# GAVLab/feature_extraction

Measured on AMD Instinct MI355X. Metric: VLP-16 scans/sec (16x1800 pts), detector+descriptor, higher is better.
Workload: dtype f32; 1 GPU; batch of 1024 synthetic VLP-16 scans (16x1800 pts, 64 uniform poles) per GPU, device-resident, preset 'launch', roll/pitch 0.02/-0.015; scans_per_gpu=1024, preset=launch, parallelism=frame-sharded x1, batches_in_flight=4

## Files before the change

feature_extraction_amd/csrc/fx_kernels.hip:

```cpp
#include <hip/hip_runtime.h>
#include <float.h>
#include <math.h>
#include <assert.h>
#include <type_traits>
#include <algorithm>

#include "fx_device.h"
#include "fx_sort_replay.h"
#include "fx_launch.h"
#include "../../include/fx.h"

#pragma clang fp contract(off)

#define FX_WG 256
#define FX_NWAVE (FX_WG / 64)

namespace {

typedef float fx_f2 __attribute__((ext_vector_type(2)));

__device__ __forceinline__ uint32_t lanes_below(unsigned long long m) {
  return __builtin_amdgcn_mbcnt_hi((uint32_t)(m >> 32), __builtin_amdgcn_mbcnt_lo((uint32_t)m, 0u));
}

// ... 3841 lines not shown
  for (uint32_t k = tid; k < K; k += NT) {
    const float4 kp = B.keypoints[(size_t)G.scan * G.P.max_keypoints + G.kb + k];
    s.kp[k] = kp;
    s.kcnt[k] = 0;
    s.kpos[k] = 0;
    s.knbr[k] = 0;
    if (G.slice == 0 && MODE != 1) B.row_kp[G.row0 + k] = kp;
    atomicMin(&s.w[GW_BOX + 0], f2ord(kp.x)), atomicMax(&s.w[GW_BOX + 1], f2ord(kp.x));
    atomicMin(&s.w[GW_BOX + 2], f2ord(kp.y)), atomicMax(&s.w[GW_BOX + 3], f2ord(kp.y));
    atomicMin(&s.w[GW_BOX + 4], f2ord(kp.z)), atomicMax(&s.w[GW_BOX + 5], f2ord(kp.z));
  }
  __syncthreads();
  GatherGrid g;
  const float kx0 = ord2f(s.w[GW_BOX + 0]), kx1 = ord2f(s.w[GW_BOX + 1]), ky0 = ord2f(s.w[GW_BOX + 2]), ky1 = ord2f(s.w[GW_BOX + 3]);
  g.bx0 = kx0 - box_margin, g.bx1 = kx1 + box_margin;
  g.by0 = ky0 - box_margin, g.by1 = ky1 + box_margin;
  g.bz0 = ord2f(s.w[GW_BOX + 4]) - box_margin, g.bz1 = ord2f(s.w[GW_BOX + 5]) + box_margin;
  const float wx = fmaxf(box_margin, (g.bx1 - g.bx0) / (float)(FX_GATHER_G - 1) * 1.0001f + 1e-6f);
  const float wy = fmaxf(box_margin, (g.by1 - g.by0) / (float)(FX_GATHER_G - 1) * 1.0001f + 1e-6f);
  g.inv_wx = 1.0f / wx, g.inv_wy = 1.0f / wy;
  g.ncx = min((int)((g.bx1 - g.bx0) * g.inv_wx) + 1, FX_GATHER_G), g.ncy = min((int)((g.by1 - g.by0) * g.inv_wy) + 1, FX_GATHER_G);
  const int ncx = g.ncx, ncy = g.ncy;
  for (uint32_t k = tid; k < K; k += NT) {
    const int cx = g.cell_x(s.kp[k].x), cy = g.cell_y(s.kp[k].y);
    for (int dy = -1; dy <= 1; ++dy)
      for (int dx = -1; dx <= 1; ++dx)
        if (cx + dx >= 0 && cx + dx < ncx && cy + dy >= 0 && cy + dy < ncy) atomicAdd(&s.cell[(cy + dy) * ncx + cx + dx], 1u);
  }
  __syncthreads();
  if (tid < 64) {
    const uint32_t n_cells = (uint32_t)(ncx * ncy), per = (n_cells + 63) / 64;
    uint32_t sum = 0;
    for (uint32_t u = 0; u < per; ++u) {
      const uint32_t ci = tid * per + u;
      sum += ci < n_cells ? s.cell[ci] : 0u;
    }
    uint32_t incl = sum;
    incl = wave_incl_scan(incl);
    uint32_t run = incl - sum;
    for (uint32_t u = 0; u < per; ++u) {
      const uint32_t ci = tid * per + u;
      if (ci < n_cells) {
        const uint32_t c = s.cell[ci];
        s.cell[ci] = run | (c << 20);
        s.cur[ci] = run;
        run += c;
      }
    }
  }
  __syncthreads();
  for (uint32_t k = tid; k < K; k += NT) {
    const int cx = g.cell_x(s.kp[k].x), cy = g.cell_y(s.kp[k].y);
    for (int dy = -1; dy <= 1; ++dy)
      for (int dx = -1; dx <= 1; ++dx)
        if (cx + dx >= 0 && cx + dx < ncx && cy + dy >= 0 && cy + dy < ncy)
          s.flat[atomicAdd(&s.cur[(cy + dy) * ncx + cx + dx], 1u)] = (uint16_t)k;
  }
  __syncthreads();
  return g;
}
template <int NT>
__device__ __forceinline__ void gather_slice_positions(const GatherWg &G) {
  const uint32_t S = gridDim.x;
  const uint32_t *cnt = G.B.gather_cnt + (size_t)G.scan * S * G.P.max_keypoints;
  uint32_t ovf_before = 0, ovf_all = 0;
  for (uint32_t k = G.tid; k < G.K; k += NT) {
    uint32_t run = 0, mine = 0;
    for (uint32_t sl = 0; sl < S; ++sl) {
      const uint32_t c = cnt[(size_t)sl * G.P.max_keypoints + k];
      const uint32_t o = run + c > G.P.list_cap ? run + c - max(run, G.P.list_cap) : 0u;
      if (sl == G.slice) mine = run;
      if (sl < G.slice) ovf_before += o;
      ovf_all += o;
      run += c;
    }
    G.s.kpos[k] = mine;
    if (G.slice == 0) G.B.s_cnt[G.row0 + k] = run;
  }
  if (ovf_before) atomicAdd(&G.s.w[GW_OVF], ovf_before);
  if (G.slice == 0 && ovf_all) atomicAdd(&G.B.ovf_cnt[G.scan], ovf_all);
  __syncthreads();
}
template <int NT, int MODE>
struct GatherStream {
  static constexpr uint32_t kTile = NT * 4;
  uint32_t lo, hi, tstep, nb_first;
  const uint32_t *near_bits;
  uint2 nb_words;
  __device__ __forceinline__ GatherStream(const GatherWg &G) {
    const uint32_t n = G.M.n;
    uint32_t chunk = (n + gridDim.x - 1) / gridDim.x;
    chunk = (chunk + kTile - 1) / kTile * kTile;
    tstep = MODE != 0 ? gridDim.x * kTile : kTile;
    lo = MODE != 0 ? G.slice * kTile : G.slice * chunk;
    hi = MODE != 0 ? n : (lo + chunk < n ? lo + chunk : n);
    near_bits = G.B.near_bits + (size_t)G.scan * G.P.near_words;
    nb_fill(G, lo);
  }
  __device__ __forceinline__ void nb_fill(const GatherWg &G, uint32_t i_first) {
    nb_first = i_first;
    const uint32_t i = i_first + G.lane * tstep;
    nb_words = make_uint2(0u, 0u);
    if (i < hi) {
      const uint32_t w = (i + G.wave * 256u) / 128u;
      nb_words = *reinterpret_cast<const uint2 *>(near_bits + w);
    }
  }
  __device__ __forceinline__ unsigned long long near_sectors(const GatherWg &G, uint32_t i0) {
    if (i0 >= hi) return 0ull;
    uint32_t t = (i0 - nb_first) / tstep;
    if (t >= 64u) nb_fill(G, i0), t = 0u;
    const uint32_t ts = (uint32_t)__builtin_amdgcn_readfirstlane((int)t);
    return (unsigned long long)(uint32_t)__builtin_amdgcn_readlane((int)nb_words.x, (int)ts) |
           ((unsigned long long)(uint32_t)__builtin_amdgcn_readlane((int)nb_words.y, (int)ts) << 32);
  }
  __device__ __forceinline__ void load_tile(const GatherWg &G, uint32_t i0, unsigned long long sect, float4 (&v)[4]) const {
#pragma unroll
    for (int u = 0; u < 4; ++u) {
      const uint32_t i = i0 + G.wave * 256 + u * 64 + G.lane;
      v[u] = make_float4(NAN, NAN, NAN, 0);
      if (((sect >> (16 * u + (G.lane >> 2))) & 1ull) && i < hi) v[u] = *reinterpret_cast<const float4 *>(G.M.pts + (size_t)i * G.M.stride_f);
    }
  }
};
__device__ __forceinline__ void hit_count(const GatherWg &G, uint32_t k) { atomicAdd(&G.s.kpos[k], 1u); }
__device__ __forceinline__ void hit_direct(const GatherWg &G, uint32_t k, const float4 &pq) {
  const uint32_t pos = G.own ? atomicAdd(&G.s.kpos[k], 1u) : atomicAdd(&G.B.s_cnt[G.row0 + k], 1u);
  if (pos < G.P.list_cap) {
    G.B.s_pts[(size_t)(G.row0 + k) * G.P.list_cap + pos] = pq;
  } else {
    const uint32_t os = G.own ? atomicAdd(&G.s.w[GW_OVF], 1u) : atomicAdd(&G.B.ovf_cnt[G.scan], 1u);
    if (os < G.P.ovf_cap) {
      G.ovf_pts[os] = pq;
      G.ovf_kp[os] = k;
    }
  }
}
__device__ __forceinline__ bool hit_staged(const GatherWg &G, uint32_t k, const float4 &pq) {
  const uint32_t slot = atomicAdd(&G.s.w[GW_STAGED], 1u);
  if (slot >= FX_GATHER_STAGE) return false;
  G.s.spt[slot] = pq;
  G.s.smeta[slot] = (k << 16) | atomicAdd(&G.s.kcnt[k], 1u);
  return true;
}
template <int NT>
__device__ __forceinline__ void gather_flush(const GatherWg &G, uint32_t staged) {
  staged = min(staged, (uint32_t)FX_GATHER_STAGE);
  for (uint32_t k = G.tid; k < G.K; k += NT) {
    const uint32_t c = G.s.kcnt[k];
    if (c) {
      const uint32_t base = atomicAdd(&G.B.s_cnt[G.row0 + k], c);
      G.s.kbase[k] = base;
      if (base + c > G.P.list_cap) {
        const uint32_t first = base < G.P.list_cap ? G.P.list_cap - base : 0u;
        G.s.kovf[k] = atomicAdd(&G.B.ovf_cnt[G.scan], c - first) - first;
      }
    }
    G.s.kcnt[k] = 0;
  }
  __syncthreads();
  for (uint32_t e = G.tid; e < staged; e += NT) {
    const uint32_t meta = G.s.smeta[e], k = meta >> 16;
    const uint32_t pos = G.s.kbase[k] + (meta & 0xffffu);
    if (pos < G.P.list_cap) {
      G.B.s_pts[(size_t)(G.row0 + k) * G.P.list_cap + pos] = G.s.spt[e];
    } else {
      const uint32_t slot = G.s.kovf[k] + (meta & 0xffffu);
      if (slot < G.P.ovf_cap) {
        G.ovf_pts[slot] = G.s.spt[e];
        G.ovf_kp[slot] = k;
      }
    }
  }
  if (G.tid == 0) G.s.w[GW_STAGED] = 0;
  __syncthreads();
}
template <int MODE>
__device__ __forceinline__ void gather_drain(const GatherWg &G, uint32_t &qn) {
  wave_sync_lds();
  for (uint32_t t = G.lane; t < qn; t += 64) {
    const float4 pq = G.s.q_pt[t];
    const uint32_t info = G.s.q_info[t], st = info & 0xfffffu, cnt = info >> 20;
    for (uint32_t e = 0; e < cnt; ++e) {
      const uint32_t k = G.s.flat[st + e];
      const float4 kp = G.s.kp[k];
      const float d2 = dist2(kp.x, kp.y, kp.z, pq.x, pq.y, pq.z);
      if (d2 < G.P.r2_support) {
        if (d2 < G.P.r2_search && MODE != 2) {
          if (G.solo && !G.passes)
            G.s.knbr[k] = 1u;
          else
            G.B.kp_nbrs[(size_t)G.scan * G.P.max_keypoints + G.kb + k] = 1u;
        }
        if (MODE == 1)
          hit_count(G, k);
        else if (G.own || !hit_staged(G, k, pq))
          hit_direct(G, k, pq);
      }
    }
  }
  wave_sync_lds();
  qn = 0;
}
template <int NT, int MODE>
__device__ __forceinline__ void gather_park(const GatherWg &G, const GatherGrid &g, const float4 &v, uint32_t i, uint32_t &qn) {
  const float rx = ((G.M.R[0] * v.x + G.M.R[1] * v.y) + G.M.R[2] * v.z) + 0.0f;
  const float ry = ((G.M.R[3] * v.x + G.M.R[4] * v.y) + G.M.R[5] * v.z) + 0.0f;
  const float rz = ((G.M.R[6] * v.x + G.M.R[7] * v.y) + G.M.R[8] * v.z) + 0.0f;
  const bool near = rx >= g.bx0 && rx <= g.bx1 && ry >= g.by0 && ry <= g.by1 && rz >= g.bz0 && rz <= g.bz1 &&
                    isfinite(rx) && isfinite(ry) && isfinite(rz);
  uint32_t info = 0;
  if (near) info = G.s.cell[g.cell_y(ry) * g.ncx + g.cell_x(rx)];
  const bool has = (info >> 20) != 0u;
  const unsigned long long m = __ballot(has);
  if (m) {
    if (has) {
      const uint32_t slot = qn + lanes_below(m);
      G.s.q_pt[slot] = make_float4(rx, ry, rz, __uint_as_float(i));
      G.s.q_info[slot] = info;
    }
    qn += (uint32_t)__popcll(m);
    if (qn > gather_queue(NT) - 64) gather_drain<MODE>(G, qn);
  }
}
template <int NT, int MODE>
__device__ __forceinline__ void gather_tail(const GatherWg &G) {
  if (MODE == 1)
    for (uint32_t k = G.tid; k < G.K; k += NT) G.B.gather_cnt[((size_t)G.scan * gridDim.x + G.slice) * G.P.max_keypoints + k] = G.s.kpos[k];
  if (G.solo) {
    for (uint32_t k = G.tid; k < G.K; k += NT) G.B.s_cnt[G.row0 + k] = G.s.kpos[k];
    for (uint32_t k0 = G.wave * 64u; k0 < G.K; k0 += NT) {
      const uint32_t k = k0 + G.lane;
      classify_rows(G.P, G.B, k < G.K, G.row0 + k, G.scan, k < G.K ? G.s.kpos[k] : 0u);
    }
    __syncthreads();
    if (G.wave == 0 && !G.passes) rng_ordinals(G.B, G.row0, G.K, G.lane, G.s.knbr);
  }
}
template <int NT, bool PASSES, int MODE = 0>
__device__ __forceinline__ void gather_body(const FxDevParams &P, const FxBuffers &B, float box_margin) {
  static_assert(MODE == 0 || !PASSES, "the counted slices hold a scan's keypoints in one pass");
  extern __shared__ __attribute__((aligned(16))) uint32_t smem[];
  const uint32_t MK = PASSES ? (uint32_t)FX_GATHER_KCAP : P.max_keypoints;
  const uint32_t scan = blockIdx.y, tid = threadIdx.x, lane = tid & 63, wave = tid >> 6;
  uint32_t K_all = B.n_kp[scan];
  if (K_all == 0) return;
  const uint32_t row_first = B.kp_offset[scan];
  if (row_first >= P.max_total_kp) return;
  if (row_first + K_all > P.max_total_kp) K_all = P.max_total_kp - row_first;
  const FxScanMeta M = B.meta[scan];
  const bool solo = gridDim.x == 1 && MODE == 0, passes = PASSES && K_all > MK;
  const GatherMem s(smem, GatherLds(MK, NT), wave, gather_queue(NT));
  if (tid == 0) s.w[GW_OVF] = 0;
  uint32_t kb = 0;
  do {
    const GatherWg G{P, B, M, s, scan, blockIdx.x, tid, lane, wave, solo, solo || MODE == 2, passes, B.ovf_pts + (size_t)scan * P.ovf_cap,
                     B.ovf_kp + (size_t)scan * P.ovf_cap, PASSES ? min(MK, K_all - kb) : K_all, kb, row_first + kb};
    const GatherGrid grid = gather_tables<NT, MODE>(G, box_margin);
    if (MODE == 2) gather_slice_positions<NT>(G);
    GatherStream<NT, MODE> st(G);
    uint32_t qn = 0;
    float4 v[4], nv[4];
    unsigned long long nib = st.near_sectors(G, st.lo), nnib = 0;
    st.load_tile(G, st.lo, nib, v);
    for (uint32_t i0 = st.lo; i0 < st.hi; i0 += st.tstep) {
      nnib = st.near_sectors(G, i0 + st.tstep);
      st.load_tile(G, i0 + st.tstep, nnib, nv);
      if (MODE == 0 && i0 != st.lo && !solo) {
        __syncthreads();
        const uint32_t staged = s.w[GW_STAGED];
        __syncthreads();
        if (staged > FX_GATHER_STAGE / 2) gather_flush<NT>(G, staged);
      }
#pragma unroll
      for (int u = 0; u < 4; ++u) {
        if (!((nib >> (16 * u)) & 0xffffull)) continue;
        gather_park<NT, MODE>(G, grid, v[u], i0 + wave * 256 + u * 64 + lane, qn);
      }
      nib = nnib;
#pragma unroll
      for (int u = 0; u < 4; ++u) v[u] = nv[u];
    }
    gather_drain<MODE>(G, qn);
    __syncthreads();
    if (MODE == 0) gather_flush<NT>(G, s.w[GW_STAGED]);
    gather_tail<NT, MODE>(G);
  } while (PASSES && (kb += MK) < K_all);
  if (solo) {
    if (tid == 0) B.ovf_cnt[scan] = s.w[GW_OVF];
    if (passes) {
      wg_global_sync();
      if (wave == 0) rng_ordinals(B, row_first, K_all, lane, B.kp_nbrs + (size_t)scan * P.max_keypoints);
    }
  }
}

extern "C" __global__ __launch_bounds__(FX_GATHER_T) void k_gather(FxDevParams P, FxBuffers B, float box_margin) { gather_body<FX_GATHER_T, false>(P, B, box_margin); }
extern "C" __global__ __launch_bounds__(FX_GATHER_WIDE_T) void k_gather_wide(FxDevParams P, FxBuffers B, float box_margin) { gather_body<FX_GATHER_WIDE_T, false>(P, B, box_margin); }
extern "C" __global__ __launch_bounds__(FX_GATHER_T) void k_gather_count(FxDevParams P, FxBuffers B, float box_margin) { gather_body<FX_GATHER_T, false, 1>(P, B, box_margin); }
extern "C" __global__ __launch_bounds__(FX_GATHER_T) void k_gather_scatter(FxDevParams P, FxBuffers B, float box_margin) { gather_body<FX_GATHER_T, false, 2>(P, B, box_margin); }
extern "C" __global__ __launch_bounds__(FX_GATHER_WIDE_T) void k_gather_passes(FxDevParams P, FxBuffers B, float box_margin) { gather_body<FX_GATHER_WIDE_T, true>(P, B, box_margin); }

#define FX_WAVE_WORDS (FX_WAVE_CAP * 8)
__device__ __forceinline__ void desc_zero_row(float *out, uint32_t lane, uint32_t stride) {
  const uint32_t head = (uint32_t)((16u - ((uintptr_t)out & 15u)) & 15u) / 4u;
  const uint32_t n4 = (FX_DESC_FLOATS - head) / 4u, tail0 = head + 4u * n4;
  if (lane < head) out[lane] = 0.0f;
  if (lane < FX_DESC_FLOATS - tail0) out[tail0 + lane] = 0.0f;
  float4 *body = reinterpret_cast<float4 *>(out + head);
  for (uint32_t t = lane; t < n4; t += stride) body[t] = make_float4(0.f, 0.f, 0.f, 0.f);
}
__device__ __forceinline__ void desc_fill_nan(float *out, uint32_t lane, uint32_t stride) {
  for (uint32_t t = lane; t < FX_DESC_FLOATS; t += stride) out[t] = t < FX_DESC_BINS ? NAN : 0.0f;
}
__device__ __forceinline__ void desc_clear_row(const FxBuffers &B, uint32_t row, uint32_t nb_prev, uint32_t lane, uint32_t stride) {
  float *out = B.desc + (size_t)row * FX_DESC_FLOATS;
  if (nb_prev > FX_GROUP_CAP) {
    desc_zero_row(out, lane, stride);
  } else {
    const uint16_t *bins = B.desc_bins + (size_t)row * FX_GROUP_CAP;
    for (uint32_t t = lane; t < nb_prev; t += stride) out[bins[t]] = 0.0f;
  }
}

#define FX_TABLE_WORDS 208
__device__ __forceinline__ const FxScTables *tables_to_lds(const FxBuffers &B, uint32_t *dst) {
  const float *src = reinterpret_cast<const float *>(B.tables);
  for (uint32_t t = threadIdx.x; t < sizeof(FxScTables) / 4; t += blockDim.x) dst[t] = __float_as_uint(src[t]);
  __syncthreads();
  return reinterpret_cast<const FxScTables *>(dst);
}

template <bool FAST>
__device__ __forceinline__ void desc_wave_body(const FxDevParams &P, const FxBuffers &B, uint32_t batch,
                                               uint32_t *smem, uint32_t bid, uint32_t nblk) {
  const uint32_t lane = threadIdx.x & 63, wave = threadIdx.x >> 6;
  const WithinR2 within(P.r2_density);
  uint32_t *base = smem + wave * FX_WAVE_WORDS;
  float4 *sp = reinterpret_cast<float4 *>(base);
  unsigned long long *nkey = reinterpret_cast<unsigned long long *>(base + 4 * FX_WAVE_CAP);
  float *nw = reinterpret_cast<float *>(base + 6 * FX_WAVE_CAP);
  uint32_t *sidx = base + 7 * FX_WAVE_CAP;
  unsigned long long *skey = reinterpret_cast<unsigned long long *>(base);
  float *sw = reinterpret_cast<float *>(base + 2 * FX_WAVE_CAP);
  const FxScTables *T = tables_to_lds(B, smem + FX_NWAVE * FX_WAVE_WORDS);

  uint32_t total = B.kp_offset[batch];
  if (total > P.max_total_kp) total = P.max_total_kp;
  const uint32_t n_items = B.counters[8];
  for (uint32_t it = bid * FX_NWAVE + wave; it < n_items; it += nblk * FX_NWAVE) {
    const uint32_t row = B.wave_desc[it];
    const uint2 rm = B.row_map[row];
    const uint32_t scan = rm.x, k = rm.y;
    const uint32_t nS = B.s_cnt[row];
    const float4 kp = B.row_kp[row];
    const float2 xa = B.row_xa[row];
    float4 lv[FX_WAVE_CAP / 64];
#pragma unroll
    for (uint32_t u = 0; u < FX_WAVE_CAP / 64; ++u)
      if (lane + u * 64 < P.list_cap) lv[u] = B.s_pts[(size_t)row * P.list_cap + lane + u * 64];
    const uint32_t nb_prev = B.desc_nbins[row];
    if (nS > FX_WAVE_CAP || nS > P.list_cap) continue;
    float *out = B.desc + (size_t)row * FX_DESC_FLOATS;
    desc_clear_row(B, row, nb_prev, lane, 64u);
    if (lane == 0) B.desc_nbins[row] = FX_ROW_DIRTY;
    __builtin_amdgcn_wave_barrier();
    uint32_t nAll = 0;
#pragma unroll
    for (uint32_t u = 0; u < FX_WAVE_CAP / 64; ++u) {
      const uint32_t e = lane + u * 64;
      float4 v = make_float4(0, 0, 0, 0);
      float d2 = INFINITY;
      if (e < nS) {
        v = lv[u];
        d2 = dist2(kp.x, kp.y, kp.z, v.x, v.y, v.z);
      }
      const bool nb = d2 < P.r2_search;
      const unsigned long long m = __ballot(nb);
      if (e < nS) {
        const uint32_t before = nAll + lanes_below(m);
        const uint32_t pos = nb ? before : nS - 1u - (e - before);
        sp[pos] = make_float4(v.x, v.y, v.z, d2);
        sidx[pos] = __float_as_uint(v.w);
      }
      nAll += (uint32_t)__popcll(m);
    }
    __builtin_amdgcn_fence(__ATOMIC_RELEASE, "wavefront");
    __builtin_amdgcn_wave_barrier();
    __builtin_amdgcn_fence(__ATOMIC_ACQUIRE, "wavefront");

    uint32_t nM = 0;
    bool amb = false;
    for (uint32_t e0 = 0; e0 < nAll; e0 += 64) {
      const uint32_t e = e0 + lane;
      const bool nb = e < nAll;
      const float4 b = nb ? sp[e] : make_float4(0, 0, 0, INFINITY);
      const float d2 = b.w;
      const bool use = nb && !sc3d_is_origin(d2);
      unsigned long long key = 0;
      float w = 0.f;
      if (use) {
        float lut;
        const uint32_t bin = sc3d_bin<FAST>(kp, b.x, b.y, b.z, d2, xa, T, lut, amb);
        const uint32_t dens = within.count(sp, 0u, nS, b.x, b.y, b.z);
        w = (1.0f / (float)dens) * lut;
        key = sc3d_key(bin, d2, sidx[e]);
      }
      const unsigned long long um = __ballot(use);
      if (use) {
        const uint32_t pos = nM + lanes_below(um);
        nkey[pos] = key;
        nw[pos] = w;
      }
      nM += (uint32_t)__popcll(um);
    }
    if (lane == 0) B.kp_nbrs[(size_t)scan * P.max_keypoints + k] = nAll;
    __builtin_amdgcn_fence(__ATOMIC_RELEASE, "workgroup");
    if (nAll == 0) {
      desc_fill_nan(out, lane, 64);
      continue;
    }
    __builtin_amdgcn_fence(__ATOMIC_RELEASE, "wavefront");
    __builtin_amdgcn_wave_barrier();
    __builtin_amdgcn_fence(__ATOMIC_ACQUIRE, "wavefront");
    for (uint32_t e0 = 0; e0 < nM; e0 += 64) {
      const uint32_t e = e0 + lane;
      if (e < nM) {
        const unsigned long long key = nkey[e];
        uint32_t rank = 0;
#pragma unroll 8
        for (uint32_t q = 0; q < nM; ++q) rank += (nkey[q] < key) ? 1u : 0u;
        skey[rank] = key;
        sw[rank] = nw[e];
      }
    }
    __builtin_amdgcn_fence(__ATOMIC_RELEASE, "wavefront");
    __builtin_amdgcn_wave_barrier();
    __builtin_amdgcn_fence(__ATOMIC_ACQUIRE, "wavefront");
    for (uint32_t e0 = 0; e0 < nM; e0 += 64) {
      const uint32_t e = e0 + lane;
      if (e >= nM) continue;
      const uint32_t bin = (uint32_t)(skey[e] >> 52);
      if (e > 0 && (uint32_t)(skey[e - 1] >> 52) == bin) continue;
      float acc = 0.0f;
      uint32_t q = e;
      do {
        acc += sw[q];
        ++q;
      } while (q < nM && (uint32_t)(skey[q] >> 52) == bin);
      out[bin] = acc;
    }
    __builtin_amdgcn_wave_barrier();
  }
}

#define FX_GROUP_SLOTS 256
#define FX_GROUP_WAVE_WORDS (FX_GROUP_SLOTS * 8 + 32)
static_assert(FX_GROUP_CAP == 64 && FX_GROUP_SLOTS == 4 * FX_GROUP_CAP, "the group tier's LDS image and the 64-slot bin record");
#ifndef FX_GROUP_UNROLL
#define FX_GROUP_UNROLL 8
#endif
#ifndef FX_GROUP_OCC
#define FX_GROUP_OCC 4
#endif
template <uint32_t LANES>
__device__ __forceinline__ uint32_t desc_group_body(const FxDevParams &P, const FxBuffers &B, uint32_t *smem, const FxScTables *T, uint32_t bid,
                                                    uint32_t nblk, uint32_t first) {
  constexpr uint32_t GROUPS = 64u / LANES, CAP = 4u * LANES;
  constexpr uint32_t CLS = LANES == 4u ? 0u : (LANES == 8u ? 1u : 2u);
  static_assert(group_class_lanes(CLS) == LANES && group_class_cap(CLS) == CAP && CAP <= FX_GROUP_CAP, "one size class an instantiation");
  const uint32_t lane = threadIdx.x & 63, wave = threadIdx.x >> 6;
  const uint32_t gl = lane % LANES, g = lane / LANES;
  const WithinR2 within(P.r2_density);
  uint32_t *wbase = smem + wave * FX_GROUP_WAVE_WORDS, *base = wbase + g * (8u * CAP);
  float4 *sp = reinterpret_cast<float4 *>(base);
  unsigned long long *nkey = reinterpret_cast<unsigned long long *>(base + 4 * CAP);
  float *nw = reinterpret_cast<float *>(base + 6 * CAP);
  uint32_t *sidx = base + 7 * CAP;
  uint32_t *cnt = wbase + 8u * FX_GROUP_SLOTS + 2u * g;
  unsigned long long *skey = reinterpret_cast<unsigned long long *>(base);
  float *sw = reinterpret_cast<float *>(base + 2 * CAP);

  const uint32_t n_rows = min(B.counters[FX_CNT_GROUP + CLS], P.max_total_kp);
  const uint32_t *list = B.group_desc + (size_t)CLS * P.max_total_kp;
  const uint32_t n_items = (n_rows + GROUPS - 1u) / GROUPS, istride = nblk * FX_NWAVE;
  const uint32_t it0 = (bid * FX_NWAVE + wave + istride - first % istride) % istride;
  if (it0 >= n_items) return first + n_items;
  auto entry = [&](uint32_t it) -> uint32_t {
    const uint32_t i = it * GROUPS + g;
    return i < n_rows ? list[i] : FX_NONE;
  };
  uint2 f_rm = make_uint2(0u, 0u);
  uint32_t f_row = FX_NONE, f_nS = 0, f_nb = 0, f_cls = FX_ROW_GROUP;
  uint2 f_pb = make_uint2(0u, 0u);
  float4 f_kp = make_float4(0, 0, 0, 0), f_lv[4];
  float2 f_xa = make_float2(1.f, 0.f);
  auto fetch = [&](uint32_t row) {
    f_row = row, f_rm = make_uint2(0u, 0u), f_pb = make_uint2(0u, 0u), f_nS = 0, f_nb = 0, f_cls = FX_ROW_GROUP;
    f_kp = make_float4(0, 0, 0, 0), f_xa = make_float2(1.f, 0.f);
#pragma unroll
    for (uint32_t u = 0; u < 4u; ++u) f_lv[u] = make_float4(0, 0, 0, 0);
    if (row != FX_NONE) {
      if (CLS == FX_GROUP_CLASSES - 1u) f_cls = B.row_class[row];
      f_rm = B.row_map[row];
      f_nS = B.s_cnt[row];
      f_kp = B.row_kp[row];
      f_xa = B.row_xa[row];
#pragma unroll
      for (uint32_t u = 0; u < 4u; ++u)
        if (gl + u * LANES < P.list_cap) f_lv[u] = B.s_pts[(size_t)row * P.list_cap + gl + u * LANES];
      f_nb = B.desc_nbins[row];
      f_pb = *reinterpret_cast<const uint2 *>(B.desc_bins + (size_t)row * FX_GROUP_CAP + 4u * gl);
    }
  };
  fetch(entry(it0));
  uint32_t row_next = entry(it0 + istride);
  __builtin_amdgcn_wave_barrier();
  for (uint32_t it = it0; it < n_items; it += istride) {
    const uint32_t row = f_row;
    const bool dense_fail = row != FX_NONE && f_cls == FX_ROW_DENSE_FAIL;
    bool live = row != FX_NONE && (dense_fail || f_nS <= CAP);
    uint32_t scan = 0, k = 0, nS = 0;
    float4 kp = make_float4(0, 0, 0, 0);
    float2 xa = make_float2(1.f, 0.f);
    float4 lv[4];
    uint32_t nb_prev = 0;
    uint2 pb = make_uint2(0u, 0u);
    if (live) {
      scan = f_rm.x, k = f_rm.y, nS = f_nS, kp = f_kp, xa = f_xa, nb_prev = f_nb, pb = f_pb;
#pragma unroll
      for (uint32_t u = 0; u < 4u; ++u) lv[u] = f_lv[u];
    }
    float *out = B.desc + (size_t)(live ? row : 0u) * FX_DESC_FLOATS;
    uint16_t *my_bins = B.desc_bins + (size_t)(live ? row : 0u) * FX_GROUP_CAP;
    if (live) {
      if (nb_prev > FX_GROUP_CAP) {
        desc_zero_row(out, gl, LANES);
      } else {
        const uint32_t t0 = 4u * gl;
        if (t0 + 0u < nb_prev) out[pb.x & 0xffffu] = 0.0f;
        if (t0 + 1u < nb_prev) out[pb.x >> 16] = 0.0f;
        if (t0 + 2u < nb_prev) out[pb.y & 0xffffu] = 0.0f;
        if (t0 + 3u < nb_prev) out[pb.y >> 16] = 0.0f;
      }
    }
    if constexpr (CAP < FX_GROUP_CAP) {
      if (live && nb_prev > CAP && nb_prev <= FX_GROUP_CAP)
        for (uint32_t t = CAP + gl; t < nb_prev; t += LANES) out[my_bins[t]] = 0.0f;
    }
    if (dense_fail) {
      __builtin_amdgcn_fence(__ATOMIC_RELEASE, "workgroup");
      desc_fill_nan(out, gl, LANES);
      if (gl == 0) {
        B.kp_nbrs[(size_t)scan * P.max_keypoints + k] = FX_NONE;
        B.desc_nbins[row] = FX_ROW_DIRTY;
      }
      live = false;
    }
    if (!live) nS = 0;
    __builtin_amdgcn_wave_barrier();
    uint32_t nAll = 0;
#pragma unroll
    for (uint32_t u = 0; u < 4u; ++u) {
      const uint32_t e = gl + u * LANES;
      float4 v = make_float4(0, 0, 0, 0);
      float d2 = INFINITY;
      if (e < nS) {
        v = lv[u];
        d2 = dist2(kp.x, kp.y, kp.z, v.x, v.y, v.z);
      }
      const bool nb = d2 < P.r2_search;
      const unsigned long long m = __ballot(nb);
      const uint32_t gm = (uint32_t)(m >> (g * LANES)) & ((1u << LANES) - 1u);
      if (e < nS) {
        const uint32_t before = nAll + (uint32_t)__popc(gm & ((1u << gl) - 1u));
        const uint32_t pos = nb ? before : nS - 1u - (e - before);
        sp[pos] = make_float4(v.x, v.y, v.z, d2);
        sidx[pos] = __float_as_uint(v.w);
      }
      nAll += (uint32_t)__popc(gm);
    }
    if (gl < 2) cnt[gl] = 0;
    if (live && gl == 0) B.kp_nbrs[(size_t)scan * P.max_keypoints + k] = nAll;
    __builtin_amdgcn_fence(__ATOMIC_RELEASE, "wavefront");
    __builtin_amdgcn_wave_barrier();
    __builtin_amdgcn_fence(__ATOMIC_ACQUIRE, "wavefront");
    for (uint32_t e = gl; e < nAll; e += LANES) {
      const float4 b = sp[e];
      const float d2 = b.w;
      if (sc3d_is_origin(d2)) continue;
      float lut;
      bool amb = false;
      const uint32_t bin = sc3d_bin<true>(kp, b.x, b.y, b.z, d2, xa, T, lut, amb);
      const uint32_t dens = within.count(sp, 0u, nS, b.x, b.y, b.z);
      const uint32_t pos = atomicAdd(&cnt[0], 1u);
      nkey[pos] = sc3d_key(bin, d2, sidx[e]);
      nw[pos] = (1.0f / (float)dens) * lut;
    }
    __builtin_amdgcn_fence(__ATOMIC_RELEASE, "wavefront");
    __builtin_amdgcn_wave_barrier();
    __builtin_amdgcn_fence(__ATOMIC_ACQUIRE, "wavefront");
    uint32_t nM = live ? cnt[0] : 0u;
    {
      uint32_t r2 = live ? row : 0u;
      asm volatile("" : "+v"(r2));
      out = B.desc + (size_t)r2 * FX_DESC_FLOATS;
      my_bins = B.desc_bins + (size_t)r2 * FX_GROUP_CAP;
    }
    __builtin_amdgcn_fence(__ATOMIC_RELEASE, "workgroup");
    if (live) {
      if (nAll == 0) {
        desc_fill_nan(out, gl, LANES);
        nM = 0;
        if (gl == 0) B.desc_nbins[row] = FX_ROW_DIRTY;
      }
    }
    unsigned long long my_key[4];
    float my_w[4];
    uint32_t my_rank[4];
#pragma unroll
    for (uint32_t u = 0; u < 4u; ++u) {
      const uint32_t e = gl + u * LANES;
      my_rank[u] = FX_NONE;
      if (e < nM) {
        my_key[u] = nkey[e];
        my_w[u] = nw[e];
        uint32_t rank = 0;
#pragma unroll FX_GROUP_UNROLL
        for (uint32_t q = 0; q < nM; ++q) rank += (nkey[q] < my_key[u]) ? 1u : 0u;
        my_rank[u] = rank;
      }
    }
    __builtin_amdgcn_fence(__ATOMIC_RELEASE, "wavefront");
    __builtin_amdgcn_wave_barrier();
    __builtin_amdgcn_fence(__ATOMIC_ACQUIRE, "wavefront");
#pragma unroll
    for (uint32_t u = 0; u < 4u; ++u)
      if (my_rank[u] != FX_NONE) {
        skey[my_rank[u]] = my_key[u];
        sw[my_rank[u]] = my_w[u];
      }
    __builtin_amdgcn_fence(__ATOMIC_RELEASE, "wavefront");
    __builtin_amdgcn_wave_barrier();
    __builtin_amdgcn_fence(__ATOMIC_ACQUIRE, "wavefront");
    fetch(row_next);
    row_next = entry(it + 2u * istride);
    for (uint32_t e = gl; e < nM; e += LANES) {
      const uint32_t bin = (uint32_t)(skey[e] >> 52);
      if (e > 0 && (uint32_t)(skey[e - 1] >> 52) == bin) continue;
      float acc = 0.0f;
      uint32_t q = e;
      do {
        acc += sw[q];
        ++q;
      } while (q < nM && (uint32_t)(skey[q] >> 52) == bin);
      out[bin] = acc;
      my_bins[atomicAdd(&cnt[1], 1u)] = (uint16_t)bin;
    }
    __builtin_amdgcn_fence(__ATOMIC_RELEASE, "wavefront");
    __builtin_amdgcn_wave_barrier();
    __builtin_amdgcn_fence(__ATOMIC_ACQUIRE, "wavefront");
    if (live && nAll != 0 && gl == 0) B.desc_nbins[row] = cnt[1];
  }
  return first + n_items;
}

struct DescLds {
  unsigned long long *nkey;
  float4 *sp;
  float *nw, *img;
  uint32_t *sidx, *s_w;
};
#define FX_DESC_WORDS_PER_POINT 8
#define FX_DGRID3 12
__device__ __forceinline__ DescLds desc_carve(uint32_t *smem, uint32_t cap) {
  DescLds L;
  L.s_w = smem;
  uint32_t *p = smem + 16;
  L.sp = (float4 *)p, p += 4 * cap;
  L.nkey = (unsigned long long *)p, p += 2 * cap;
  L.nw = (float *)p, p += cap;
  L.sidx = p, p += cap;
  L.img = (float *)p;
  return L;
}

__device__ __forceinline__ DescLds desc_carve_gs(uint32_t *smem, uint32_t *gs, uint32_t cap) {
  DescLds L;
  L.s_w = smem;
  L.img = (float *)(smem + 16);
  uint32_t *p = gs;
  L.sp = (float4 *)p, p += 4 * (size_t)cap;
  L.nkey = (unsigned long long *)p, p += 2 * (size_t)cap;
  L.nw = (float *)p, p += cap;
  L.sidx = p;
  return L;
}

template <bool FAST, int NT, bool GS = false>
__device__ __forceinline__ bool desc_body(const FxDevParams &P, const FxBuffers &B, uint32_t row, uint32_t scan, uint32_t k,
                          uint32_t cap, uint32_t *smem, bool from_list, uint32_t *gs = nullptr) {
  DescLds L = GS ? desc_carve_gs(smem, gs, cap) : desc_carve(smem, cap);
  FX_STAMP_INIT(B.stamps && FAST ? B.stamps + 48 : nullptr);
  const uint32_t tid = threadIdx.x;
  const WithinR2 within(P.r2_density);
  const FxScanMeta M = B.meta[scan];
  const float4 kp = B.keypoints[(size_t)scan * P.max_keypoints + k];
  float *out = B.desc + (size_t)row * FX_DESC_FLOATS;
  constexpr uint32_t kPre = 4;
  const bool pre = from_list && !GS;
  float4 lv[kPre];
  uint32_t nS_pre = 0;
  float2 xa_pre = make_float2(1.f, 0.f);
  if (pre) {
    nS_pre = B.s_cnt[row];
    xa_pre = B.row_xa[row];
#pragma unroll
    for (uint32_t u = 0; u < kPre; ++u)
      if (tid + u * NT < P.list_cap) lv[u] = B.s_pts[(size_t)row * P.list_cap + tid + u * NT];
  }

  desc_clear_row(B, row, B.desc_nbins[row], tid, NT);

  if (tid < 4) L.s_w[tid] = 0;
  uint32_t *tl = reinterpret_cast<uint32_t *>(L.img) + FX_DGRID3 * FX_DGRID3 * FX_DGRID3;
  for (uint32_t t = tid; t < sizeof(FxScTables) / 4; t += NT) tl[t] = __float_as_uint(reinterpret_cast<const float *>(B.tables)[t]);
  wg_sync<GS>();
  if (tid == 0) B.desc_nbins[row] = FX_ROW_DIRTY;
  uint32_t nS;
  constexpr uint32_t G = FX_DGRID3, kCells = G * G * G;
  uint32_t *cell_end = reinterpret_cast<uint32_t *>(L.img);
  const float r_sup = sqrtf(P.r2_support);
  const float cell_w = fmaxf(sqrtf(P.r2_density) * 1.001f, 2.0f * r_sup / (float)(G - 1) * 1.0001f);
  const float inv_cw = 1.0f / cell_w, gx0 = kp.x - r_sup, gy0 = kp.y - r_sup, gz0 = kp.z - r_sup;
  auto cell_1d = [&](float v, float v0) { return (uint32_t)min(max((int)floorf((v - v0) * inv_cw), 0), (int)G - 1); };
  auto cell_of = [&](float x, float y, float z) { return (cell_1d(z, gz0) * G + cell_1d(y, gy0)) * G + cell_1d(x, gx0); };
  bool grid = false;
  if (from_list) {
    nS = pre ? nS_pre : B.s_cnt[row];
    grid = nS <= cap;
    const bool in_regs = pre && nS <= kPre * NT;
    if (grid) {
      const float4 *lst = B.s_pts + (size_t)row * P.list_cap;
      for (uint32_t t = tid; t < kCells; t += NT) cell_end[t] = 0;
      wg_sync<GS>();
      if (in_regs) {
#pragma unroll
        for (uint32_t u = 0; u < kPre; ++u)
          if (tid + u * NT < nS) atomicAdd(&cell_end[cell_of(lv[u].x, lv[u].y, lv[u].z)], 1u);
      } else {
        for (uint32_t e = tid; e < nS; e += NT) {
          const float4 v = lst[e];
          atomicAdd(&cell_end[cell_of(v.x, v.y, v.z)], 1u);
        }
      }
      wg_sync<GS>();
      if (tid < 64) {
        constexpr uint32_t per = (kCells + 63) / 64;
        uint32_t sum = 0;
        for (uint32_t u = 0; u < per; ++u) {
          const uint32_t ci = tid * per + u;
          sum += ci < kCells ? cell_end[ci] : 0u;
        }
        uint32_t incl = sum;
        incl = wave_incl_scan(incl);
        uint32_t run = incl - sum;
        for (uint32_t u = 0; u < per; ++u) {
          const uint32_t ci = tid * per + u;
          if (ci < kCells) {
            const uint32_t c = cell_end[ci];
            cell_end[ci] = run;
            run += c;
          }
        }
      }
      wg_sync<GS>();
      if (in_regs) {
#pragma unroll
        for (uint32_t u = 0; u < kPre; ++u)
          if (tid + u * NT < nS) {
            const float4 v = lv[u];
            const uint32_t slot = atomicAdd(&cell_end[cell_of(v.x, v.y, v.z)], 1u);
            L.sp[slot] = make_float4(v.x, v.y, v.z, dist2(kp.x, kp.y, kp.z, v.x, v.y, v.z));
            L.sidx[slot] = __float_as_uint(v.w);
          }
      } else {
        for (uint32_t e = tid; e < nS; e += NT) {
          const float4 v = lst[e];
          const uint32_t slot = atomicAdd(&cell_end[cell_of(v.x, v.y, v.z)], 1u);
          L.sp[slot] = make_float4(v.x, v.y, v.z, dist2(kp.x, kp.y, kp.z, v.x, v.y, v.z));
          L.sidx[slot] = __float_as_uint(v.w);
        }
      }
    } else {
      for (uint32_t e = tid; e < nS; e += NT) {
        const float4 v = B.s_pts[(size_t)row * P.list_cap + e];
        L.sp[e] = make_float4(v.x, v.y, v.z, dist2(kp.x, kp.y, kp.z, v.x, v.y, v.z));
        L.sidx[e] = __float_as_uint(v.w);
      }
    }
    wg_sync<GS>();
  } else {
    const uint32_t n = M.n;
    for (uint32_t i0 = 0; i0 < n; i0 += NT * 4) {
      float4 v[4];
#pragma unroll
      for (int u = 0; u < 4; ++u) {
        const uint32_t i = i0 + u * NT + tid;
        v[u] = i < n ? *reinterpret_cast<const float4 *>(M.pts + (size_t)i * M.stride_f) : make_float4(NAN, NAN, NAN, 0);
      }
#pragma unroll
      for (int u = 0; u < 4; ++u) {
        const float x = v[u].x, y = v[u].y, z = v[u].z;
        const float rx = ((M.R[0] * x + M.R[1] * y) + M.R[2] * z) + 0.0f;
        const float ry = ((M.R[3] * x + M.R[4] * y) + M.R[5] * z) + 0.0f;
        const float rz = ((M.R[6] * x + M.R[7] * y) + M.R[8] * z) + 0.0f;
        const float d = dist2(kp.x, kp.y, kp.z, rx, ry, rz);
        if (d < P.r2_support && isfinite(rx) && isfinite(ry) && isfinite(rz)) {
          const uint32_t pos = atomicAdd(&L.s_w[0], 1u);
          if (pos < cap) {
            L.sp[pos] = make_float4(rx, ry, rz, d);
            L.sidx[pos] = i0 + u * NT + tid;
          }
        }
      }
    }
    wg_sync<GS>();
    nS = L.s_w[0];
    if (nS > cap) return false;
  }
  FX_STAMP(1);

  const FxScTables *T = reinterpret_cast<const FxScTables *>(tl);
  const float2 xa = pre ? xa_pre : B.row_xa[row];
  uint32_t *nlist = reinterpret_cast<uint32_t *>(L.nw);
  uint32_t *dens = reinterpret_cast<uint32_t *>(L.nkey);
  {
    uint32_t *scratch = reinterpret_cast<uint32_t *>(L.img) + FX_DESC_BINS - 32;
    uint32_t n_use = 0;
    for (uint32_t e0 = 0; e0 < nS; e0 += NT) {
      const uint32_t e = e0 + tid;
      const float d2 = e < nS ? L.sp[e].w : INFINITY;
      const bool nb = d2 < P.r2_search, use = nb && !sc3d_is_origin(d2);
      const unsigned long long m_nb = __ballot(nb);
      if ((tid & 63u) == 0 && m_nb) atomicAdd(&L.s_w[2], (uint32_t)__popcll(m_nb));
      uint32_t tot;
      const uint32_t r = block_rank<NT>(use, scratch, tot);
      if (use) {
        nlist[n_use + r] = e;
        dens[2 * (n_use + r)] = 0u;
      }
      n_use += tot;
    }
    if (tid == 0) L.s_w[1] = n_use;
  }
  wg_sync<GS>();
  FX_STAMP(6);
  {
    const uint32_t nMq = L.s_w[1];
    uint32_t parts = 1;
    while (parts < (grid ? 8u : 32u) && nMq * parts * 2 <= (uint32_t)NT) parts <<= 1;
    const uint32_t chunk = (nS + parts - 1) / parts;
    for (uint32_t t = tid; t < nMq * parts; t += NT) {
      const uint32_t m = t / parts, part = t % parts;
      const float4 bq = L.sp[nlist[m]];
      uint32_t c = 0;
      if (grid) {
        const uint32_t cx = cell_1d(bq.x, gx0), cy = cell_1d(bq.y, gy0), cz = cell_1d(bq.z, gz0);
        const uint32_t xa0 = cx > 0 ? cx - 1 : 0, xa1 = min(cx + 1, G - 1);
        for (uint32_t rowi = part; rowi < 9; rowi += parts) {
          const uint32_t yy = cy + rowi % 3u - 1u, zz = cz + rowi / 3u - 1u;
          if (yy >= G || zz >= G) continue;
          const uint32_t c0 = (zz * G + yy) * G + xa0, c1 = (zz * G + yy) * G + xa1;
          const uint32_t q0 = c0 ? cell_end[c0 - 1] : 0u, q1 = cell_end[c1];
          c += within.count(L.sp, q0, q1, bq.x, bq.y, bq.z);
        }
      } else {
        const uint32_t q0 = part * chunk, q1 = min(q0 + chunk, nS);
        c += within.count(L.sp, q0, q1, bq.x, bq.y, bq.z);
      }
      if (c) atomicAdd(&dens[2 * m], c);
    }
    wg_sync<GS>();
    FX_STAMP(7);
    for (uint32_t m = tid; m < nMq; m += NT) {
      const uint32_t e = nlist[m];
      const float4 bq = L.sp[e];
      float lut;
      bool amb = false;
      const uint32_t bin = sc3d_bin<FAST>(kp, bq.x, bq.y, bq.z, bq.w, xa, T, lut, amb);
      const uint32_t d = dens[2 * m];
      L.nkey[m] = sc3d_key(bin, bq.w, L.sidx[e]);
      L.nw[m] = (1.0f / (float)d) * lut;
    }
  }
  __builtin_amdgcn_fence(__ATOMIC_RELEASE, "workgroup");
  wg_sync<GS>();
  FX_STAMP(2);
  for (uint32_t t = tid; t < FX_DESC_BINS; t += NT) L.img[t] = 0.0f;
  const uint32_t nM = L.s_w[1], nAll = L.s_w[2];
  if (tid == 0) {
    FX_COUNT(12, 1);
    FX_COUNT(13, nS);
    FX_COUNT(14, nM);
  }
  if (tid == 0) B.kp_nbrs[(size_t)scan * P.max_keypoints + k] = nAll;
  if (nAll == 0) {
    desc_fill_nan(out, tid, NT);
    wg_sync<GS>();
    return true;
  }
  uint32_t *bin_end = reinterpret_cast<uint32_t *>(L.img);
  unsigned long long *skey = reinterpret_cast<unsigned long long *>(L.sp);
  float *sw = reinterpret_cast<float *>(L.sp) + 2 * cap;
  float *sorted_w = reinterpret_cast<float *>(L.sp) + 3 * cap;
  wg_sync<GS>();
  for (uint32_t m = tid; m < nM; m += NT) atomicAdd(&bin_end[(uint32_t)(L.nkey[m] >> 52)], 1u);
  wg_sync<GS>();
  if (tid < 64) {
    constexpr uint32_t per = (FX_DESC_BINS + 63) / 64;
    uint32_t sum = 0;
    for (uint32_t u = 0; u < per; ++u) {
      const uint32_t bi = tid * per + u;
      sum += bi < FX_DESC_BINS ? bin_end[bi] : 0u;
    }
    uint32_t incl = sum;
    incl = wave_incl_scan(incl);
    uint32_t run = incl - sum;
    for (uint32_t u = 0; u < per; ++u) {
      const uint32_t bi = tid * per + u;
      if (bi < FX_DESC_BINS) {
        const uint32_t c = bin_end[bi];
        bin_end[bi] = run;
        run += c;
      }
    }
  }
  wg_sync<GS>();
  for (uint32_t m = tid; m < nM; m += NT) {
    const unsigned long long key = L.nkey[m];
    const uint32_t pos = atomicAdd(&bin_end[(uint32_t)(key >> 52)], 1u);
    skey[pos] = key;
    sw[pos] = L.nw[m];
  }
  wg_sync<GS>();
  for (uint32_t p = tid; p < nM; p += NT) {
    const unsigned long long key = skey[p];
    const uint32_t bin = (uint32_t)(key >> 52);
    const uint32_t s0 = bin ? bin_end[bin - 1u] : 0u, s1 = bin_end[bin];
    uint32_t rank = 0;
    for (uint32_t q = s0; q < s1; ++q) rank += skey[q] < key ? 1u : 0u;
    sorted_w[s0 + rank] = sw[p];
  }
  wg_sync<GS>();
  FX_STAMP(3);
  for (uint32_t bin = tid; bin < FX_DESC_BINS; bin += NT) {
    const uint32_t s0 = bin ? bin_end[bin - 1u] : 0u, s1 = bin_end[bin];
    if (s0 == s1) continue;
    float acc = 0.0f;
    for (uint32_t q = s0; q < s1; ++q) acc += sorted_w[q];
    out[bin] = acc;
  }
  wg_sync<GS>();
  FX_STAMP(4);
  FX_STAMP(5);
// ... 1411 lines not shown
```

Baseline: 2.329 million scans/s.

## Deal group-tier neighbor items across the whole wave to balance per-group work

In the grouped descriptor kernel, each lane group previously processed only its own keypoint's neighbors, so lanes idled when group neighbor counts differed. The new code builds a wave-wide prefix scan of per-group neighbor counts, writes a deal list of (group, element) items and per-group context (keypoint, axis, counts, row) to extra LDS, and lets all 64 lanes process items for any group. Per-group state is then reloaded from LDS after the barrier. This adds LDS footprint per wave, a scan, and indirect LDS addressing, which may reduce occupancy or add latency.

```diff
diff --git a/feature_extraction_amd/csrc/fx_kernels.hip b/feature_extraction_amd/csrc/fx_kernels.hip
--- a/feature_extraction_amd/csrc/fx_kernels.hip
+++ b/feature_extraction_amd/csrc/fx_kernels.hip
@@ -4167,13 +4167,13 @@
 extern "C" __global__ __launch_bounds__(FX_GATHER_WIDE_T) void k_gather_passes(FxDevParams P, FxBuffers B, float box_margin) { gather_body<FX_GATHER_WIDE_T, true>(P, B, box_margin); }
 
 #define FX_WAVE_WORDS (FX_WAVE_CAP * 8)
-__device__ __forceinline__ void desc_zero_row(float *out, uint32_t lane, uint32_t stride) {
+__device__ __forceinline__ void desc_zero_row(float *out, uint32_t lane, uint32_t stride, float zero = 0.0f) {
   const uint32_t head = (uint32_t)((16u - ((uintptr_t)out & 15u)) & 15u) / 4u;
   const uint32_t n4 = (FX_DESC_FLOATS - head) / 4u, tail0 = head + 4u * n4;
   if (lane < head) out[lane] = 0.0f;
   if (lane < FX_DESC_FLOATS - tail0) out[tail0 + lane] = 0.0f;
   float4 *body = reinterpret_cast<float4 *>(out + head);
-  for (uint32_t t = lane; t < n4; t += stride) body[t] = make_float4(0.f, 0.f, 0.f, 0.f);
+  for (uint32_t t = lane; t < n4; t += stride) body[t] = make_float4(zero, zero, zero, zero);
 }
 __device__ __forceinline__ void desc_fill_nan(float *out, uint32_t lane, uint32_t stride) {
   for (uint32_t t = lane; t < FX_DESC_FLOATS; t += stride) out[t] = t < FX_DESC_BINS ? NAN : 0.0f;
@@ -4320,7 +4320,7 @@
 }
 
 #define FX_GROUP_SLOTS 256
-#define FX_GROUP_WAVE_WORDS (FX_GROUP_SLOTS * 8 + 32)
+#define FX_GROUP_WAVE_WORDS (FX_GROUP_SLOTS * 8 + 32 + 8 * 16 + FX_GROUP_SLOTS / 2)
 static_assert(FX_GROUP_CAP == 64 && FX_GROUP_SLOTS == 4 * FX_GROUP_CAP, "the group tier's LDS image and the 64-slot bin record");
 #ifndef FX_GROUP_UNROLL
 #define FX_GROUP_UNROLL 8
@@ -4343,6 +4343,8 @@
   float *nw = reinterpret_cast<float *>(base + 6 * CAP);
   uint32_t *sidx = base + 7 * CAP;
   uint32_t *cnt = wbase + 8u * FX_GROUP_SLOTS + 2u * g;
+  float4 *rctx = reinterpret_cast<float4 *>(wbase + 8u * FX_GROUP_SLOTS + 32u);
+  uint16_t *deal = reinterpret_cast<uint16_t *>(wbase + 8u * FX_GROUP_SLOTS + 32u + 8u * 16u);
   unsigned long long *skey = reinterpret_cast<unsigned long long *>(base);
   float *sw = reinterpret_cast<float *>(base + 2 * CAP);
 
@@ -4400,7 +4402,9 @@
     uint16_t *my_bins = B.desc_bins + (size_t)(live ? row : 0u) * FX_GROUP_CAP;
     if (live) {
       if (nb_prev > FX_GROUP_CAP) {
-        desc_zero_row(out, gl, LANES);
+        float zero = 0.0f;
+        asm volatile("" : "+v"(zero));
+        desc_zero_row(out, gl, LANES, zero);
       } else {
         const uint32_t t0 = 4u * gl;
         if (t0 + 0u < nb_prev) out[pb.x & 0xffffu] = 0.0f;
@@ -4447,37 +4451,54 @@
     }
     if (gl < 2) cnt[gl] = 0;
     if (live && gl == 0) B.kp_nbrs[(size_t)scan * P.max_keypoints + k] = nAll;
+    const uint32_t incl = wave_incl_scan(gl == 0u ? nAll : 0u);
+    const uint32_t n_deal = (uint32_t)__builtin_amdgcn_readlane((int)incl, 63);
+    if (gl == 0u) {
+      rctx[2u * g] = make_float4(kp.x, kp.y, kp.z, __uint_as_float(nS));
+      rctx[2u * g + 1u] = make_float4(xa.x, xa.y, __uint_as_float(nAll), __uint_as_float(live ? row : FX_NONE));
+    }
+#pragma unroll
+    for (uint32_t u = 0; u < 4u; ++u) {
+      const uint32_t e = gl + u * LANES;
+      if (e < nAll) deal[incl - nAll + e] = (uint16_t)((g << 8) | e);
+    }
     __builtin_amdgcn_fence(__ATOMIC_RELEASE, "wavefront");
     __builtin_amdgcn_wave_barrier();
     __builtin_amdgcn_fence(__ATOMIC_ACQUIRE, "wavefront");
-    for (uint32_t e = gl; e < nAll; e += LANES) {
-      const float4 b = sp[e];
+    for (uint32_t t = lane; t < n_deal; t += 64u) {
+      const uint32_t item = deal[t], q = item >> 8, e = item & 0xffu;
+      uint32_t *qbase = wbase + q * (8u * CAP);
+      const float4 *qsp = reinterpret_cast<const float4 *>(qbase);
+      const float4 b = qsp[e];
       const float d2 = b.w;
       if (sc3d_is_origin(d2)) continue;
+      const float4 qkp = rctx[2u * q];
+      const float4 qxa = rctx[2u * q + 1u];
       float lut;
       bool amb = false;
-      const uint32_t bin = sc3d_bin<true>(kp, b.x, b.y, b.z, d2, xa, T, lut, amb);
-      const uint32_t dens = within.count(sp, 0u, nS, b.x, b.y, b.z);
-      const uint32_t pos = atomicAdd(&cnt[0], 1u);
-      nkey[pos] = sc3d_key(bin, d2, sidx[e]);
-      nw[pos] = (1.0f / (float)dens) * lut;
+      const uint32_t bin = sc3d_bin<true>(qkp, b.x, b.y, b.z, d2, make_float2(qxa.x, qxa.y), T, lut, amb);
+      const uint32_t dens = within.count(qsp, 0u, __float_as_uint(qkp.w), b.x, b.y, b.z);
+      const uint32_t pos = atomicAdd(wbase + 8u * FX_GROUP_SLOTS + 2u * q, 1u);
+      reinterpret_cast<unsigned long long *>(qbase + 4u * CAP)[pos] = sc3d_key(bin, d2, (qbase + 7u * CAP)[e]);
+      reinterpret_cast<float *>(qbase + 6u * CAP)[pos] = (1.0f / (float)dens) * lut;
     }
     __builtin_amdgcn_fence(__ATOMIC_RELEASE, "wavefront");
     __builtin_amdgcn_wave_barrier();
     __builtin_amdgcn_fence(__ATOMIC_ACQUIRE, "wavefront");
-    uint32_t nM = live ? cnt[0] : 0u;
+    const uint32_t nAll_b = __float_as_uint(rctx[2u * g + 1u].z), row_b = __float_as_uint(rctx[2u * g + 1u].w);
+    const bool live_b = row_b != FX_NONE;
+    uint32_t nM = live_b ? cnt[0] : 0u;
     {
-      uint32_t r2 = live ? row : 0u;
-      asm volatile("" : "+v"(r2));
+      const uint32_t r2 = live_b ? row_b : 0u;
       out = B.desc + (size_t)r2 * FX_DESC_FLOATS;
       my_bins = B.desc_bins + (size_t)r2 * FX_GROUP_CAP;
     }
     __builtin_amdgcn_fence(__ATOMIC_RELEASE, "workgroup");
-    if (live) {
-      if (nAll == 0) {
+    if (live_b) {
+      if (nAll_b == 0) {
         desc_fill_nan(out, gl, LANES);
         nM = 0;
-        if (gl == 0) B.desc_nbins[row] = FX_ROW_DIRTY;
+        if (gl == 0) B.desc_nbins[row_b] = FX_ROW_DIRTY;
       }
     }
     unsigned long long my_key[4];
@@ -4525,7 +4546,7 @@
     __builtin_amdgcn_fence(__ATOMIC_RELEASE, "wavefront");
     __builtin_amdgcn_wave_barrier();
     __builtin_amdgcn_fence(__ATOMIC_ACQUIRE, "wavefront");
-    if (live && nAll != 0 && gl == 0) B.desc_nbins[row] = cnt[1];
+    if (live_b && nAll_b != 0 && gl == 0) B.desc_nbins[row_b] = cnt[1];
   }
   return first + n_items;
 }
```

Measured after the change: 2.336 million scans/s, median of 2. Within noise of the previous version (+0.3%).
